# WarranWeng/ESR

Hardware: AMD Instinct MI355X
Metric: SR event-frames/sec (whole node), 2x NFS-syn (higher is better)
Workload: dtype bf16; 1 GPU; model=ESRNet-basech8, global_batch=64, seq_len=8, seqn=3, window_events=2048, input=128x128->256x256, scale=2, upsampler=pixelshuffle, hip_graphs=full, parallelism=dp1

## Files before the change

### esr_amd/ops/conv.py

```python

from __future__ import annotations

import os

import torch
import torch.nn.functional as F

from .native import get_ext

__all__ = ["conv2d_act", "native_conv_supported", "ACT_IDS"]

ACT_IDS = {None: 0, "none": 0, "relu": 1, "sigmoid": 2, "tanh": 3}

stats = {"native_calls": 0, "native_calls_fp16": 0, "native_bias_grad": 0}

_MFMA_MIN_COUT = 32
_CIK = 32


_FP16_DEFAULT = "1"


_BIAS_GRAD_DEFAULT = "native"


def _enabled() -> bool:
    return os.environ.get("ESR_NATIVE_CONV", "1") != "0"


def _native_bias_grad() -> bool:
    return os.environ.get("ESR_BIAS_GRAD", _BIAS_GRAD_DEFAULT) != "aten"


def native_fp16_enabled() -> bool:
    return os.environ.get("ESR_NATIVE_FP16", _FP16_DEFAULT) != "0"


def compute_dtype(autocast_on: bool, autocast_dtype, x_dtype,
                  fp16_enabled: bool | None = None):
    dt = autocast_dtype if autocast_on else x_dtype
    if dt == torch.bfloat16:
        return torch.bfloat16
    if dt == torch.float16:
        if fp16_enabled is None:
            fp16_enabled = native_fp16_enabled()
        return torch.float16 if fp16_enabled else None
    return None


def _ceil(v: int, m: int) -> int:
    return (v + m - 1) // m * m


def _pack(w: torch.Tensor) -> torch.Tensor:
    O, I, k, _ = w.shape
    t = w.permute(2, 3, 0, 1).reshape(k * k, O, I)
    op, ip = _ceil(O, 16), _ceil(I, _CIK)
    if op != O or ip != I:
        t = F.pad(t, (0, ip - I, 0, op - O))
    return t.contiguous()


class _NativeConv2dFn(torch.autograd.Function):
    @staticmethod
    def forward(ctx, x, w, bias, stride, act_id):
        ext = get_ext()
        ks = w.shape[2]
        cout, cin = w.shape[0], w.shape[1]
        bias_f = bias.float() if bias is not None else None
        if cout >= _MFMA_MIN_COUT:
            y = ext.conv2d_fwd_mfma(x, _pack(w), bias_f, cout, ks, stride,
                                    act_id)
        elif cin < _MFMA_MIN_COUT and x.shape[-1] % 8 == 0:
            y = ext.conv2d_fwd_valu2(x, w.contiguous(), bias_f, stride,
                                     act_id)
        else:
            y = ext.conv2d_fwd_valu(x, w.contiguous(), bias_f, stride, act_id)
        ctx.save_for_backward(x, w, y)
        ctx.stride_ = stride
        ctx.act_id = act_id
        ctx.has_bias = bias is not None
        return y

    @staticmethod
    def backward(ctx, dy):
        ext = get_ext()
        x, w, y = ctx.saved_tensors
        stride, act_id = ctx.stride_, ctx.act_id
        ks = w.shape[2]
        cout, cin = w.shape[0], w.shape[1]
        dy = dy.contiguous()
        fused_db = ctx.has_bias and _native_bias_grad()
        db = None
        if fused_db:
            stats["native_bias_grad"] += 1
            if act_id:
                dpre, db = ext.act_grad_bias(dy, y, act_id)[:2]
            else:
                dpre, db = dy, ext.bias_grad(dy)[0]
        else:
            dpre = ext.act_grad(dy, y, act_id) if act_id else dy
        aten_db = ctx.has_bias and not fused_db

        mode = os.environ.get("ESR_CONV_BWD", "aten")
        native_bwd = mode == "native" or (
            mode == "auto" and stride == 1 and cin >= _MFMA_MIN_COUT)
        if x.dtype != torch.bfloat16:
            native_bwd = False
        if not native_bwd:
            dx, dw, db_aten = torch.ops.aten.convolution_backward(
                dpre, x, w, [cout] if aten_db else None,
                [stride, stride], [ks // 2, ks // 2], [1, 1], False, [0, 0],
                1, [True, True, aten_db])
            return dx, dw, db_aten if aten_db else db, None, None

        if stride == 1:
            wt = w.transpose(0, 1)
            if ks == 3:
                wt = wt.flip((2, 3))
            if cin >= _MFMA_MIN_COUT:
                dx = ext.conv2d_fwd_mfma(dpre, _pack(wt), None, cin, ks, 1, 0)
            else:
                dx = ext.conv2d_fwd_valu(dpre, wt.contiguous(), None, 1, 0)
        else:
            dx = ext.conv2d_dgrad_s2(dpre, w.contiguous(),
                                     x.shape[2], x.shape[3])

        dwp = ext.conv2d_wgrad_mfma(x, dpre, ks, stride,
                                    _ceil(cin, 16), _ceil(cout, 16))
        dw = dwp.permute(1, 0, 2, 3)[:cout, :cin].to(w.dtype)
        if aten_db:
            db = dpre.sum(dim=(0, 2, 3), dtype=torch.float32).to(w.dtype)
        return dx, dw, db, None, None


def shape_supported(conv: torch.nn.Conv2d, dtype=None) -> bool:
    if conv.out_channels < _MFMA_MIN_COUT and conv.in_channels < _MFMA_MIN_COUT:
        if conv.stride[0] != 1:
            return False
    if dtype == torch.float16:
        if conv.out_channels < _MFMA_MIN_COUT <= conv.in_channels:
            return False
        if conv.out_channels >= 128 and conv.kernel_size == (3, 3) \
                and conv.stride == (1, 1):
            return False
    if conv.groups != 1 or conv.dilation != (1, 1):
        return False
    kh, kw = conv.kernel_size
    sh, sw = conv.stride
    ph, pw = conv.padding if isinstance(conv.padding, tuple) else \
        (conv.padding, conv.padding)
    if kh != kw or sh != sw or ph != pw:
        return False
    if (kh, sh) not in ((3, 1), (3, 2), (1, 1)):
        return False
    if ph != kh // 2:
        return False
    return True


def native_conv_supported(x: torch.Tensor, conv: torch.nn.Conv2d,
                          dtype=None) -> bool:
    if not (_enabled() and x.is_cuda and get_ext() is not None):
        return False
    return shape_supported(conv, dtype)


def conv2d_act(x: torch.Tensor, conv: torch.nn.Conv2d, act: str | None):
    if act not in ACT_IDS or not (x.is_cuda and _enabled()):
        return None
    autocast_on = torch.is_autocast_enabled()
    dt = compute_dtype(
        autocast_on,
        torch.get_autocast_dtype("cuda") if autocast_on else None, x.dtype)
    if dt is None or not native_conv_supported(x, conv, dt):
        return None
    if x.dtype != dt:
        x = x.to(dt)
    w, b = conv.weight, conv.bias
    if w.dtype != dt:
        w = w.to(dt)
        if b is not None:
            b = b.to(dt)
    stats["native_calls"] += 1
    if dt == torch.float16:
        stats["native_calls_fp16"] += 1
# ... 3 lines not shown
```

### esr_amd/ops/native/src/bindings.cpp

```cpp
#include <torch/extension.h>

at::Tensor deform_conv2d_forward(
    const at::Tensor&, const at::Tensor&, const at::Tensor&,
    const at::Tensor&, const c10::optional<at::Tensor>&,
    int64_t, int64_t, int64_t, int64_t, int64_t, int64_t, int64_t);
std::vector<at::Tensor> deform_conv2d_backward(
    const at::Tensor&, const at::Tensor&, const at::Tensor&,
    const at::Tensor&, const at::Tensor&,
    int64_t, int64_t, int64_t, int64_t, int64_t, int64_t, int64_t);
std::vector<at::Tensor> deform_conv2d_forward_cols(
    const at::Tensor&, const at::Tensor&, const at::Tensor&,
    const at::Tensor&, const c10::optional<at::Tensor>&,
    int64_t, int64_t, int64_t, int64_t, int64_t, int64_t, int64_t);
std::vector<at::Tensor> deform_conv2d_backward_cols(
    const at::Tensor&, const at::Tensor&, const at::Tensor&,
    const at::Tensor&, const at::Tensor&, const c10::optional<at::Tensor>&,
    int64_t, int64_t, int64_t, int64_t, int64_t, int64_t, int64_t,
    const std::string&);
at::Tensor deform_conv2d_forward_fused(
    const at::Tensor&, const at::Tensor&, const at::Tensor&,
    const at::Tensor&, const c10::optional<at::Tensor>&, int64_t);
at::Tensor deform_im2col_debug(
    const at::Tensor&, const at::Tensor&, const at::Tensor&,
    int64_t, int64_t, int64_t, int64_t, int64_t, int64_t, int64_t, int64_t,
    int64_t);

std::vector<at::Tensor> gru_gates_ur_forward(const at::Tensor&,
                                             const at::Tensor&);
std::vector<at::Tensor> gru_gates_ur_backward(
    const at::Tensor&, const at::Tensor&, const at::Tensor&,
    const at::Tensor&, const at::Tensor&, const at::Tensor&);
std::vector<at::Tensor> gru_gates_out_forward(const at::Tensor&,
                                              const at::Tensor&,
                                              const at::Tensor&);
std::vector<at::Tensor> gru_gates_out_backward(
    const at::Tensor&, const at::Tensor&, const at::Tensor&,
    const at::Tensor&);

at::Tensor splat_count(const at::Tensor&, int64_t, int64_t);
at::Tensor splat_stack(const at::Tensor&, int64_t, int64_t, int64_t, double,
                       double);
int64_t grid_cap();

at::Tensor conv2d_fwd_mfma(const at::Tensor&, const at::Tensor&,
                           const c10::optional<at::Tensor>&,
                           int64_t, int64_t, int64_t, int64_t);
at::Tensor conv2d_fwd_valu(const at::Tensor&, const at::Tensor&,
                           const c10::optional<at::Tensor>&, int64_t, int64_t);
at::Tensor conv2d_fwd_valu2(const at::Tensor&, const at::Tensor&,
                            const c10::optional<at::Tensor>&, int64_t, int64_t);
at::Tensor conv2d_dgrad_s2(const at::Tensor&, const at::Tensor&,
                           int64_t, int64_t);
at::Tensor conv2d_wgrad_mfma(const at::Tensor&, const at::Tensor&,
                             int64_t, int64_t, int64_t, int64_t);
at::Tensor act_grad(const at::Tensor&, const at::Tensor&, int64_t);
std::vector<at::Tensor> act_grad_bias(const at::Tensor&, const at::Tensor&,
                                      int64_t, bool);
std::vector<at::Tensor> bias_grad(const at::Tensor&, bool);
int64_t bias_grad_chain(int64_t, int64_t, int64_t);
int64_t bias_grad_chunk();
at::Tensor gemm16_probe(const at::Tensor&, const at::Tensor&);

std::vector<at::Tensor> redistribute_stack_hip(const at::Tensor&, int64_t,
                                               int64_t, int64_t, int64_t);

void flat_grad_finite_check(const at::Tensor&, at::Tensor&);
void flat_adam_step(at::Tensor&, const at::Tensor&, at::Tensor&, at::Tensor&,
                    const c10::optional<at::Tensor>&, const at::Tensor&,
                    double, double, double, double, bool);
void flat_scale_update(at::Tensor&, bool, double, double, int64_t, double,
                       double);
void flat_grad_stats(const at::Tensor&, at::Tensor&, at::Tensor&, at::Tensor&,
                     double);
void flat_adam_step_clipped(at::Tensor&, const at::Tensor&, at::Tensor&,
                            at::Tensor&, const c10::optional<at::Tensor>&,
                            const at::Tensor&, const at::Tensor&, double,
                            double, double, double, bool);

void stream_window_advance(at::Tensor&, const at::Tensor&);
void stream_splat_ragged(const at::Tensor&, const at::Tensor&,
                         const at::Tensor&, at::Tensor&, int64_t);

void evs_batch_splat(const at::Tensor&, const at::Tensor&, at::Tensor&,
                     int64_t, int64_t, int64_t);
int64_t evs_batch_splat_chunk();

at::Tensor restoration_metrics(const at::Tensor&, const at::Tensor&, double);
std::vector<int64_t> restoration_metrics_tile();

std::vector<at::Tensor> sr_emit_scratch(const at::Tensor&, int64_t, int64_t);
at::Tensor sr_emit_counts(const at::Tensor&, int64_t);
void sr_emit_window(const at::Tensor&, const at::Tensor&,
                    const std::vector<at::Tensor>&, at::Tensor&, int64_t,
                    int64_t, int64_t, int64_t,
                    const std::vector<at::Tensor>&);

PYBIND11_MODULE(TORCH_EXTENSION_NAME, m) {
  m.def("deform_conv2d_forward", &deform_conv2d_forward,
        "modulated deformable conv forward (gfx950)");
  m.def("deform_conv2d_backward", &deform_conv2d_backward,
        "modulated deformable conv backward (gfx950, batched)");
  m.def("deform_conv2d_forward_cols", &deform_conv2d_forward_cols,
        "im2col + GEMM forward; returns (out, cols) for the backward to reuse");
  m.def("deform_conv2d_backward_cols", &deform_conv2d_backward_cols,
        "backward with optional saved columns and a path selector "
        "(auto / fused / split)");
  m.def("deform_im2col", &deform_im2col_debug,
        "deformable im2col (test hook)");
  m.def("deform_conv2d_forward_fused", &deform_conv2d_forward_fused,
        "fused im2col+MFMA deformable conv forward (test hook)");
  m.def("gru_gates_ur_forward", &gru_gates_ur_forward);
  m.def("gru_gates_ur_backward", &gru_gates_ur_backward);
  m.def("gru_gates_out_forward", &gru_gates_out_forward);
  m.def("gru_gates_out_backward", &gru_gates_out_backward);
  m.def("splat_count", &splat_count);
  m.def("splat_stack", &splat_stack);
  m.def("grid_cap", &grid_cap,
        "work items one grid of a capped grid-stride kernel covers");
  m.def("conv2d_fwd_mfma", &conv2d_fwd_mfma,
        "bf16/fp16 NCHW conv fwd, MFMA implicit GEMM, fused bias+act (gfx950)");
  m.def("conv2d_fwd_valu", &conv2d_fwd_valu,
        "bf16/fp16 NCHW conv fwd, direct VALU, fused bias+act (gfx950)");
  m.def("conv2d_fwd_valu2", &conv2d_fwd_valu2,
        "bf16/fp16 NCHW conv fwd, register-strip VALU v2 for tiny channels");
  m.def("conv2d_dgrad_s2", &conv2d_dgrad_s2,
        "bf16 stride-2 conv input-grad (gfx950)");
  m.def("conv2d_wgrad_mfma", &conv2d_wgrad_mfma,
        "bf16 conv weight-grad, MFMA split-K + fp32 atomics (gfx950)");
  m.def("act_grad", &act_grad, "fused activation backward (bf16/fp16)");
  m.def("act_grad_bias", &act_grad_bias,
        "activation backward + per-channel bias grad in one pass: "
        "{dpre, db}, with want_f32 also the fp32 sums; deterministic "
        "(bf16/fp16)",
        py::arg("dy"), py::arg("y"), py::arg("act"),
        py::arg("want_f32") = false);
  m.def("bias_grad", &bias_grad,
        "per-channel sum of an NCHW gradient: {db}, with want_f32 also the "
        "fp32 sums; deterministic (bf16/fp16)",
        py::arg("dy"), py::arg("want_f32") = false);
  m.def("bias_grad_chunk", &bias_grad_chunk,
        "elements of a channel one block of bias_grad sums");
  m.def("bias_grad_chain", &bias_grad_chain,
        "longest fp32 addition chain of bias_grad for (B, H, W)");
  m.def("gemm16_probe", &gemm16_probe, "16x16x32 bf16/fp16 MFMA fragment probe");
  m.def("redistribute_stack_hip", &redistribute_stack_hip,
        "count stack -> sorted event cloud, device-only "
        "(scan + scatter + segmented radix sort)");
  m.def("flat_grad_finite_check", &flat_grad_finite_check,
        "raise found_inf in the device state if the flat fp32 grad has "
        "inf/NaN");
  m.def("flat_adam_step", &flat_adam_step,
        "flat-buffer Adam/AdamW step with device-side un-scale and skip");
  m.def("flat_scale_update", &flat_scale_update,
        "GradScaler-style scale/step update of the device state");
  m.def("flat_grad_stats", &flat_grad_stats,
        "finite check plus deterministic fp64 sum of squares of the flat "
        "grad; writes grad norm, clip coefficient and clipped-step count");
  m.def("flat_adam_step_clipped", &flat_adam_step_clipped,
        "flat_adam_step with the gradient multiplied by the clip "
        "coefficient after un-scaling");
  m.def("stream_window_advance", &stream_window_advance,
        "per-stream sliding-window shift/reset of a [seqn,S,2,kH,kW] buffer, "
        "control read from a device tensor");
  m.def("stream_splat_ragged", &stream_splat_ragged,
        "splat concatenated per-stream LR event windows into the newest "
        "frame of a [seqn,S,2,kH,kW] buffer");
  m.def("evs_batch_splat", &evs_batch_splat,
        "splat a batch of packed event windows (jobs read from a device "
        "tensor) into [J,2,kH,kW] count planes, in place");
  m.def("evs_batch_splat_chunk", &evs_batch_splat_chunk,
        "events one block of evs_batch_splat covers");
  m.def("restoration_metrics", &restoration_metrics,
        "per-plane sum|p-t|, sum(p-t)^2, max t, min t and 7x7 SSIM sum of "
        "fp32 [P,H,W] maps, fp64 [P,5], deterministic");
  m.def("restoration_metrics_tile", &restoration_metrics_tile,
        "(TH, TW) pixel tile one block of restoration_metrics owns");
  m.def("sr_emit_scratch", &sr_emit_scratch,
        "scratch of sr_emit_window for (ncells, capacity), allocated once");
  m.def("sr_emit_counts", &sr_emit_counts,
        "the counts stage of sr_emit_window: NaN -> 0, else "
        "clamp(rint(v), 0, cell_cap), int32 (test hook)");
// ... 7 lines not shown
```

### esr_amd/ops/native/src/conv2d.hip

```cpp

#include <torch/extension.h>
#include <ATen/hip/HIPContext.h>
#include "esr_common.h"

namespace {

using s16x8 = __attribute__((ext_vector_type(8))) short;
using f32x4 = __attribute__((ext_vector_type(4))) float;

constexpr int TW = 32;
constexpr int TH = 2;
constexpr int CIK = 32;
constexpr int SLOT = 40;

template <int ACT> ESR_INLINE float apply_act(float v);
template <> ESR_INLINE float apply_act<0>(float v) { return v; }
template <> ESR_INLINE float apply_act<1>(float v) { return v > 0.f ? v : 0.f; }
template <> ESR_INLINE float apply_act<2>(float v) { return esr_sigmoid(v); }
template <> ESR_INLINE float apply_act<3>(float v) { return tanhf(v); }

ESR_INLINE float bf16u_to_f(ushort u) {
  unsigned int x = (unsigned int)u << 16;
  return __uint_as_float(x);
}
// ... 76 lines not shown
        for (int c = 0; c < CIK; ++c)
          vals[c] = (c < cmax) ? src[c * plane] : (ushort)0;
      } else {
#pragma unroll
        for (int c = 0; c < CIK; ++c) vals[c] = 0;
      }
#pragma unroll
      for (int v = 0; v < CIK / 8; ++v)
        *reinterpret_cast<s16x8*>(&patch[p * SLOT + v * 8]) =
            *reinterpret_cast<const s16x8*>(&vals[v * 8]);
    }
    __syncthreads();

#pragma unroll
    for (int tap = 0; tap < KS * KS; ++tap) {
      const int ky = tap / KS, kx = tap % KS;
      s16x8 a[MREP];
#pragma unroll
      for (int m = 0; m < MREP; ++m) {
        int row = co0 + wm * 16 * MREP + m * 16 + (lane & 15);
        row = row < Cout_p ? row : Cout_p - 1;
        a[m] = *reinterpret_cast<const s16x8*>(
            &wp[((long long)tap * Cout_p + row) * Cin_p + ci0 + kgrp]);
      }
#pragma unroll
      for (int nf = 0; nf < 2; ++nf) {
        const int pidx = wn * 32 + nf * 16 + (lane & 15);
        const int py = (pidx >> 5) * STRIDE + ky;
        const int px = (pidx & 31) * STRIDE + kx;
        const s16x8 bfrag = *reinterpret_cast<const s16x8*>(
            &patch[(py * PW + px) * SLOT + kgrp]);
#pragma unroll
        for (int m = 0; m < MREP; ++m)
          acc[m][nf] = E::mfma(a[m], bfrag, acc[m][nf]);
      }
    }
  }

#pragma unroll
  for (int m = 0; m < MREP; ++m) {
#pragma unroll
    for (int nf = 0; nf < 2; ++nf) {
      const int pidx = wn * 32 + nf * 16 + (lane & 15);
      const int oy = ty0 + (pidx >> 5), ox = tx0 + (pidx & 31);
      if (oy >= Ho || ox >= Wo) continue;
#pragma unroll
      for (int j = 0; j < 4; ++j) {
        const int co = co0 + wm * 16 * MREP + m * 16 + (lane >> 4) * 4 + j;
        if (co >= Cout) continue;
        float v = acc[m][nf][j];
        if (bias) v += bias[co];
        v = apply_act<ACT>(v);
        y[(((long long)b * Cout + co) * Ho + oy) * Wo + ox] = E::from_f(v);
      }
    }
  }
}


template <typename E, int KS, int STRIDE, int ACT>
__global__ void conv2d_fwd_valu_kernel(
    long long n, const ushort* __restrict__ x,
    const ushort* __restrict__ w,
    const float* __restrict__ bias, ushort* __restrict__ y,
    int Cin, int H, int W, int Cout, int Ho, int Wo) {
  constexpr int PAD = KS / 2;
  ESR_KERNEL_LOOP(i, n) {
    const int ox = (int)(i % Wo);
    long long t = i / Wo;
    const int oy = (int)(t % Ho); t /= Ho;
    const int co = (int)(t % Cout);
    const int b = (int)(t / Cout);
    const long long plane = (long long)H * W;
    const ushort* xb = x + (long long)b * Cin * plane;
    const ushort* wc = w + (long long)co * Cin * KS * KS;
    float acc = bias ? bias[co] : 0.f;
    const int iy0 = oy * STRIDE - PAD, ix0 = ox * STRIDE - PAD;
    for (int ci = 0; ci < Cin; ++ci) {
      const ushort* xp = xb + ci * plane;
      const ushort* wk = wc + ci * KS * KS;
#pragma unroll
      for (int ky = 0; ky < KS; ++ky) {
        const int iy = iy0 + ky;
        if (iy < 0 || iy >= H) continue;
#pragma unroll
        for (int kx = 0; kx < KS; ++kx) {
          const int ix = ix0 + kx;
          if (ix < 0 || ix >= W) continue;
          acc += E::to_f(xp[(long long)iy * W + ix]) *
                 E::to_f(wk[ky * KS + kx]);
        }
      }
    }
    y[i] = E::from_f(apply_act<ACT>(acc));
  }
}


template <typename E, int KS, int STRIDE, int ACT, int COCH>
__global__ __launch_bounds__(256)
void conv2d_fwd_valu2_kernel(
    const ushort* __restrict__ x,
    const ushort* __restrict__ w,
    const float* __restrict__ bias, ushort* __restrict__ y,
    int Cin, int H, int W, int Cout, int Ho, int Wo,
    long long nstrips, int nsx) {
// ... 362 lines not shown
            const int slot = KS == 1 ? oy % NSLOT
                : (((oy + ky - PAD) % NSLOT) + NSLOT) % NSLOT;
#pragma unroll
            for (int nci = 0; nci < 2; ++nci) {
              const s16x8 bfrag = *reinterpret_cast<const s16x8*>(
                  &xs[((nci * 16 + (lane & 15)) * NSLOT + slot) * WGV2_XW
                      + kgrp]);
#pragma unroll
              for (int kx = 0; kx < KS; ++kx)
                acc[ky * KS + kx][nci] =
                    __builtin_amdgcn_mfma_f32_16x16x32_bf16(
                        afrag[kx], bfrag, acc[ky * KS + kx][nci], 0, 0, 0);
            }
          }
        }
      }
      __syncthreads();
    }
  }

  if (abl == 1) return;
  float* part = dwp + ((((long long)blockIdx.x * gridDim.y + blockIdx.y)
                        * gridDim.z + blockIdx.z) * (32 * 64 * NTAP));
#pragma unroll
  for (int tap = 0; tap < NTAP; ++tap) {
#pragma unroll
    for (int nci = 0; nci < 2; ++nci) {
#pragma unroll
      for (int j = 0; j < 4; ++j) {
        const int co = wave * 16 + (lane >> 4) * 4 + j;
        const int ci = nci * 16 + (lane & 15);
        part[((long long)ci * 64 + co) * NTAP + tap] = acc[tap][nci][j];
      }
    }
  }
}

template <int NTAP>
__global__ void conv2d_wgrad_reduce_kernel(
    long long n, const float* __restrict__ part, int ng, int ciblks,
    int coblks, int Cin_p, int Cout_p, float* __restrict__ dwp) {
  ESR_KERNEL_LOOP(i, n) {
    const int tap = (int)(i % NTAP);
    const int co = (int)((i / NTAP) % Cout_p);
    const int ci = (int)(i / ((long long)NTAP * Cout_p));
    const int cib = ci / 32, cob = co / 64;
    const long long base =
        ((long long)cib * coblks + cob) * (32 * 64 * NTAP)
        + (((long long)(ci % 32) * 64 + (co % 64)) * NTAP + tap);
    const long long gstride = (long long)ciblks * coblks * (32 * 64 * NTAP);
    float v = 0.f;
    for (int g = 0; g < ng; ++g) v += part[g * gstride + base];
    dwp[i] = v;
  }
}


template <int ACT> ESR_INLINE float act_grad_value(float g, float v) {
  if (ACT == 0) return g;
  if (ACT == 1) return v > 0.f ? g : 0.f;
  if (ACT == 2) return g * v * (1.f - v);
  return g * (1.f - v * v);
}

template <typename E, int ACT>
ESR_INLINE ushort act_grad_elem(ushort dy, ushort y) {
  float d = act_grad_value<ACT>(E::to_f(dy), E::to_f(y));
  asm("" : "+v"(d));
  return E::from_f(d);
}

template <typename E, int ACT>
__global__ void act_grad_kernel(long long n, const ushort* __restrict__ dy,
                                const ushort* __restrict__ y,
                                ushort* __restrict__ dpre) {
  ESR_KERNEL_LOOP(i, n) {
    dpre[i] = act_grad_elem<E, ACT>(dy[i], y[i]);
  }
}


constexpr int BG_VPT = 2;
constexpr int BG_CHUNK = ESR_BLOCK * BG_VPT * 8;

ESR_INLINE float bg_block_sum(float v, float* red) {
#pragma unroll
  for (int off = 32; off > 0; off >>= 1) v += __shfl_down(v, off, 64);
  const int lane = threadIdx.x & 63, wave = threadIdx.x >> 6;
  __syncthreads();
  if (lane == 0) red[wave] = v;
  __syncthreads();
  return ((red[0] + red[1]) + red[2]) + red[3];
}

template <typename E, int ACT, bool STORE>
__global__ __launch_bounds__(ESR_BLOCK)
void act_grad_bias_kernel(int C, unsigned int HW, unsigned int L,
                          unsigned int P, bool vec,
                          const ushort* __restrict__ dy,
                          const ushort* __restrict__ y,
                          ushort* __restrict__ dpre,
                          float* __restrict__ part) {
  __shared__ float red[ESR_BLOCK / 64];
  const long long nitem = (long long)C * P;
  for (long long item = blockIdx.x; item < nitem; item += gridDim.x) {
    const int c = (int)(item / P);
// ... 128 lines not shown
  if (!bias.has_value()) return nullptr;
  TORCH_CHECK(bias->scalar_type() == at::kFloat && bias->is_contiguous() &&
              bias->device() == x.device(),
              "bias: contiguous fp32 tensor on x's device required, got ",
              bias->scalar_type());
  return bias->data_ptr<float>();
}

at::Tensor conv2d_fwd_mfma(const at::Tensor& x, const at::Tensor& wp,
                           const c10::optional<at::Tensor>& bias,
                           int64_t Cout, int64_t ks, int64_t stride,
                           int64_t act) {
  check_16bit(x, "conv2d_fwd_mfma: x");
  check_16bit(wp, "conv2d_fwd_mfma: wp");
  check_same_dtype(x, wp, "conv2d_fwd_mfma: x / wp");
  TORCH_CHECK(x.dim() == 4 && wp.dim() == 3,
              "x [B,Cin,H,W], wp: packed [ntap,Cop,Cip]");
  const int B = x.size(0), Cin = x.size(1), H = x.size(2), W = x.size(3);
  const int Cout_p = wp.size(1), Cin_p = wp.size(2);
  TORCH_CHECK(wp.size(0) == ks * ks && Cin_p % CIK == 0 && Cout_p % 16 == 0);
  const int Ho = (H + 2 * (int)(ks / 2) - (int)ks) / (int)stride + 1;
  const int Wo = (W + 2 * (int)(ks / 2) - (int)ks) / (int)stride + 1;
  auto y = at::empty({B, Cout, Ho, Wo}, x.options());
  const float* bias_ptr = bias_ptr_f32(bias, x);
  const int mrep = (Cout > 32 && Cout_p % 32 == 0) ? 2 : 1;
  const int ntx = (Wo + TW - 1) / TW, nty = (Ho + TH - 1) / TH;
  dim3 grid(ntx * nty, B, (Cout_p + 32 * mrep - 1) / (32 * mrep));
  auto stream = at::hip::getCurrentHIPStream();
  DISPATCH_ELEM(x.scalar_type(), [&] {
  DISPATCH_KS_STRIDE((int)ks, (int)stride, [&] {
    DISPATCH_ACT((int)act, [&] {
      if (mrep == 2)
        hipLaunchKernelGGL((conv2d_fwd_mfma_kernel<elem_t, kKS, kST, kAct, 2>),
                           grid, dim3(256), 0, stream,
                           (const ushort*)x.data_ptr(), (const ushort*)wp.data_ptr(),
                           bias_ptr, (ushort*)y.data_ptr(),
                           Cin, H, W, (int)Cout, Ho, Wo, Cin_p, Cout_p, ntx);
      else
        hipLaunchKernelGGL((conv2d_fwd_mfma_kernel<elem_t, kKS, kST, kAct, 1>),
                           grid, dim3(256), 0, stream,
                           (const ushort*)x.data_ptr(), (const ushort*)wp.data_ptr(),
                           bias_ptr, (ushort*)y.data_ptr(),
                           Cin, H, W, (int)Cout, Ho, Wo, Cin_p, Cout_p, ntx);
      return 0;
    });
    return 0;
  });
  return 0;
  });
  C10_HIP_KERNEL_LAUNCH_CHECK();
  return y;
}

at::Tensor conv2d_fwd_valu(const at::Tensor& x, const at::Tensor& w,
                           const c10::optional<at::Tensor>& bias,
                           int64_t stride, int64_t act) {
  check_16bit(x, "conv2d_fwd_valu: x");
  check_16bit(w, "conv2d_fwd_valu: w");
  check_same_dtype(x, w, "conv2d_fwd_valu: x / w");
  const int B = x.size(0), Cin = x.size(1), H = x.size(2), W = x.size(3);
  const int Cout = w.size(0), ks = w.size(2);
  const int Ho = (H + 2 * (ks / 2) - ks) / (int)stride + 1;
  const int Wo = (W + 2 * (ks / 2) - ks) / (int)stride + 1;
  auto y = at::empty({B, Cout, Ho, Wo}, x.options());
  const float* bias_ptr = bias_ptr_f32(bias, x);
  const long long n = (long long)B * Cout * Ho * Wo;
  auto stream = at::hip::getCurrentHIPStream();
  DISPATCH_ELEM(x.scalar_type(), [&] {
  DISPATCH_KS_STRIDE(ks, (int)stride, [&] {
    DISPATCH_ACT((int)act, [&] {
      hipLaunchKernelGGL((conv2d_fwd_valu_kernel<elem_t, kKS, kST, kAct>),
                         dim3(esr_grid(n)), dim3(ESR_BLOCK), 0, stream,
                         n, (const ushort*)x.data_ptr(), (const ushort*)w.data_ptr(),
                         bias_ptr, (ushort*)y.data_ptr(), Cin, H, W, Cout, Ho, Wo);
      return 0;
    });
    return 0;
  });
  return 0;
  });
  C10_HIP_KERNEL_LAUNCH_CHECK();
  return y;
}

at::Tensor conv2d_fwd_valu2(const at::Tensor& x, const at::Tensor& w,
                            const c10::optional<at::Tensor>& bias,
                            int64_t stride, int64_t act) {
  check_16bit(x, "conv2d_fwd_valu2: x");
  check_16bit(w, "conv2d_fwd_valu2: w");
  check_same_dtype(x, w, "conv2d_fwd_valu2: x / w");
  const int B = x.size(0), Cin = x.size(1), H = x.size(2), W = x.size(3);
  const int Cout = w.size(0), ks = w.size(2);
  TORCH_CHECK(Cin <= 32, "valu2 is for tiny-channel shapes (Cin <= 32)");
  const int Ho = (H + 2 * (ks / 2) - ks) / (int)stride + 1;
  const int Wo = (W + 2 * (ks / 2) - ks) / (int)stride + 1;
  auto y = at::empty({B, Cout, Ho, Wo}, x.options());
  const float* bias_ptr = bias_ptr_f32(bias, x);
  const int coch = Cout >= 8 || Cout > 2 ? 8 : 2;
  const int nsx = (Wo + 7) / 8;
  const long long nstrips = (long long)B * Ho * nsx;
  dim3 grid(esr_grid(nstrips), 1, (Cout + coch - 1) / coch);
  auto stream = at::hip::getCurrentHIPStream();
  DISPATCH_ELEM(x.scalar_type(), [&] {
  DISPATCH_KS_STRIDE(ks, (int)stride, [&] {
    DISPATCH_ACT((int)act, [&] {
      if (coch == 8)
        hipLaunchKernelGGL((conv2d_fwd_valu2_kernel<elem_t, kKS, kST, kAct, 8>),
                           grid, dim3(256), 0, stream,
                           (const ushort*)x.data_ptr(),
                           (const ushort*)w.data_ptr(), bias_ptr,
                           (ushort*)y.data_ptr(), Cin, H, W, Cout, Ho, Wo,
                           nstrips, nsx);
      else
        hipLaunchKernelGGL((conv2d_fwd_valu2_kernel<elem_t, kKS, kST, kAct, 2>),
                           grid, dim3(256), 0, stream,
                           (const ushort*)x.data_ptr(),
                           (const ushort*)w.data_ptr(), bias_ptr,
                           (ushort*)y.data_ptr(), Cin, H, W, Cout, Ho, Wo,
                           nstrips, nsx);
      return 0;
    });
    return 0;
  });
  return 0;
  });
  C10_HIP_KERNEL_LAUNCH_CHECK();
  return y;
}

at::Tensor conv2d_dgrad_s2(const at::Tensor& dy, const at::Tensor& w,
                           int64_t H, int64_t W) {
  check_bf16_4d(dy, "conv2d_dgrad_s2: dy");
  check_bf16_4d(w, "conv2d_dgrad_s2: w");
  const int B = dy.size(0), Cout = dy.size(1), Ho = dy.size(2), Wo = dy.size(3);
  const int Cin = w.size(1), ks = w.size(2);
  TORCH_CHECK(ks == 3, "dgrad_s2 supports 3x3 only");
  auto dx = at::empty({B, Cin, H, W}, dy.options());
  const long long n = (long long)B * Cin * H * W;
  auto stream = at::hip::getCurrentHIPStream();
  hipLaunchKernelGGL((conv2d_dgrad_s2_valu_kernel<3>),
                     dim3(esr_grid(n)), dim3(ESR_BLOCK), 0, stream,
                     n, (const ushort*)dy.data_ptr(), (const ushort*)w.data_ptr(),
                     (ushort*)dx.data_ptr(), Cin, (int)H, (int)W, Cout, Ho, Wo);
  C10_HIP_KERNEL_LAUNCH_CHECK();
  return dx;
}

at::Tensor conv2d_wgrad_mfma(const at::Tensor& x, const at::Tensor& dpre,
                             int64_t ks, int64_t stride,
                             int64_t Cin_p, int64_t Cout_p) {
  check_bf16_4d(x, "conv2d_wgrad: x");
  check_bf16_4d(dpre, "conv2d_wgrad: dpre");
  const int B = x.size(0), Cin = x.size(1), H = x.size(2), W = x.size(3);
  const int Cout = dpre.size(1), Ho = dpre.size(2), Wo = dpre.size(3);
  TORCH_CHECK(Cin_p % 16 == 0 && Cout_p % 16 == 0);
  auto dwp = at::zeros({Cin_p, Cout_p, ks, ks},
                       x.options().dtype(at::kFloat));
  const int uw = (W + TW - 1) / TW;
  auto stream = at::hip::getCurrentHIPStream();
  if (stride == 1) {
    const int ciblks = (Cin_p + 31) / 32, coblks = (Cout_p + 63) / 64;
    long long nb = (long long)B * uw * ciblks * coblks;
    int fpb = 1;
    while (fpb < 32 && fpb * 2 <= B && nb / (fpb * 2) >= 1024) fpb *= 2;
    static const int abl = [] {
      const char* e = getenv("ESR_WGRAD_ABL");
      return e ? atoi(e) : 0;
    }();
    const int bblks = (B + fpb - 1) / fpb;
    const int ng = bblks * uw;
    const int ntap = (int)(ks * ks);
    dim3 grid((unsigned)ng, ciblks, coblks);
    auto part = at::empty({(long long)ng * ciblks * coblks * 32 * 64 * ntap},
                          x.options().dtype(at::kFloat));
    if (ks == 3)
      hipLaunchKernelGGL((conv2d_wgrad_s1_kernel<3>), grid, dim3(256), 0,
                         stream, (const ushort*)x.data_ptr(),
                         (const ushort*)dpre.data_ptr(),
                         part.data_ptr<float>(),
                         Cin, H, W, Cout, (int)Cin_p, (int)Cout_p, uw, B,
                         fpb, abl);
    else
      hipLaunchKernelGGL((conv2d_wgrad_s1_kernel<1>), grid, dim3(256), 0,
                         stream, (const ushort*)x.data_ptr(),
                         (const ushort*)dpre.data_ptr(),
                         part.data_ptr<float>(),
                         Cin, H, W, Cout, (int)Cin_p, (int)Cout_p, uw, B,
                         fpb, abl);
    const long long nred = (long long)Cin_p * Cout_p * ntap;
    if (ks == 3)
      hipLaunchKernelGGL((conv2d_wgrad_reduce_kernel<9>),
                         dim3(esr_grid(nred)), dim3(ESR_BLOCK), 0, stream,
                         nred, part.data_ptr<float>(), ng, ciblks, coblks,
                         (int)Cin_p, (int)Cout_p, dwp.data_ptr<float>());
    else
      hipLaunchKernelGGL((conv2d_wgrad_reduce_kernel<1>),
                         dim3(esr_grid(nred)), dim3(ESR_BLOCK), 0, stream,
                         nred, part.data_ptr<float>(), ng, ciblks, coblks,
                         (int)Cin_p, (int)Cout_p, dwp.data_ptr<float>());
  } else {
    const int rows_per_blk = 16;
    const long long nslab =
        (long long)B * ((Ho + rows_per_blk - 1) / rows_per_blk) * uw;
    dim3 grid((unsigned)nslab, Cin_p / 16, Cout_p / 16);
    TORCH_CHECK(ks == 3, "stride-2 wgrad supports 3x3 only");
    hipLaunchKernelGGL((conv2d_wgrad_mfma_kernel<3, 2>),
                       grid, dim3(256), 0, stream,
                       (const ushort*)x.data_ptr(), (const ushort*)dpre.data_ptr(),
                       dwp.data_ptr<float>(), Cin, H, W, Cout, Ho, Wo,
                       (int)Cin_p, (int)Cout_p, rows_per_blk);
  }
  C10_HIP_KERNEL_LAUNCH_CHECK();
  return dwp;
}

at::Tensor act_grad(const at::Tensor& dy, const at::Tensor& y, int64_t act) {
  check_16bit(dy, "act_grad: dy");
  check_16bit(y, "act_grad: y");
  check_same_dtype(dy, y, "act_grad: dy / y");
  TORCH_CHECK(dy.numel() == y.numel(), "act_grad: dy and y sizes differ");
  auto dpre = at::empty_like(dy);
  const long long n = dy.numel();
  auto stream = at::hip::getCurrentHIPStream();
  DISPATCH_ELEM(dy.scalar_type(), [&] {
  DISPATCH_ACT((int)act, [&] {
    if (kAct == 0) { dpre.copy_(dy); return 0; }
    hipLaunchKernelGGL((act_grad_kernel<elem_t, kAct>),
                       dim3(esr_grid(n)), dim3(ESR_BLOCK), 0, stream,
                       n, (const ushort*)dy.data_ptr(),
                       (const ushort*)y.data_ptr(), (ushort*)dpre.data_ptr());
    return 0;
  });
  return 0;
  });
  C10_HIP_KERNEL_LAUNCH_CHECK();
  return dpre;
}

int64_t bias_grad_chunk() { return BG_CHUNK; }

int64_t bias_grad_chain(int64_t B, int64_t H, int64_t W) {
// ... 98 lines not shown
```

Measured before the change: 3099 frames/s.

## Add stride-1 MFMA conv core and route deep convs' forward and backward natively

Result: faster. 3605 frames/s (median of 6 runs) (+16.3%).

```diff
diff --git a/esr_amd/ops/conv.py b/esr_amd/ops/conv.py
--- a/esr_amd/ops/conv.py
+++ b/esr_amd/ops/conv.py
@@ -22,6 +22,12 @@
 
 
 _BIAS_GRAD_DEFAULT = "native"
+
+
+_CONV_BWD_DEFAULT = "auto"
+_AUTO_WGRAD_MIN_CIN = 192
+
+_CONV_FWD_DEFAULT = "auto"
 
 
 def _enabled() -> bool:
@@ -68,7 +74,10 @@
         ks = w.shape[2]
         cout, cin = w.shape[0], w.shape[1]
         bias_f = bias.float() if bias is not None else None
-        if cout >= _MFMA_MIN_COUT:
+        if fwd_core_route(os.environ.get("ESR_CONV_FWD", _CONV_FWD_DEFAULT),
+                          x.dtype == torch.bfloat16, ks, stride, cin, cout):
+            y = ext.conv2d_s1(x, w.contiguous(), bias_f, act_id, False)
+        elif cout >= _MFMA_MIN_COUT:
             y = ext.conv2d_fwd_mfma(x, _pack(w), bias_f, cout, ks, stride,
                                     act_id)
         elif cin < _MFMA_MIN_COUT and x.shape[-1] % 8 == 0:
@@ -102,36 +111,63 @@
             dpre = ext.act_grad(dy, y, act_id) if act_id else dy
         aten_db = ctx.has_bias and not fused_db
 
-        mode = os.environ.get("ESR_CONV_BWD", "aten")
-        native_bwd = mode == "native" or (
-            mode == "auto" and stride == 1 and cin >= _MFMA_MIN_COUT)
-        if x.dtype != torch.bfloat16:
-            native_bwd = False
-        if not native_bwd:
+        dgrad_native, wgrad_native = bwd_route(
+            os.environ.get("ESR_CONV_BWD", _CONV_BWD_DEFAULT),
+            x.dtype == torch.bfloat16, ks, stride, cin, cout)
+        pad = [ks // 2, ks // 2]
+        if not (dgrad_native and wgrad_native):
             dx, dw, db_aten = torch.ops.aten.convolution_backward(
                 dpre, x, w, [cout] if aten_db else None,
-                [stride, stride], [ks // 2, ks // 2], [1, 1], False, [0, 0],
-                1, [True, True, aten_db])
-            return dx, dw, db_aten if aten_db else db, None, None
-
-        if stride == 1:
-            wt = w.transpose(0, 1)
-            if ks == 3:
-                wt = wt.flip((2, 3))
-            if cin >= _MFMA_MIN_COUT:
-                dx = ext.conv2d_fwd_mfma(dpre, _pack(wt), None, cin, ks, 1, 0)
+                [stride, stride], pad, [1, 1], False, [0, 0], 1,
+                [not dgrad_native, not wgrad_native, aten_db])
+            if aten_db:
+                db = db_aten
+        elif aten_db:
+            db = dpre.sum(dim=(0, 2, 3), dtype=torch.float32).to(w.dtype)
+
+        if dgrad_native:
+            if stride == 1 and cin >= _MFMA_MIN_COUT:
+                dx = ext.conv2d_s1(dpre, w.contiguous(), None, 0, True)
+            elif stride == 1:
+                wt = w.transpose(0, 1)
+                if ks == 3:
+                    wt = wt.flip((2, 3))
+                dx = ext.conv2d_fwd_valu(dpre, wt.contiguous(), None, 1, 0)
             else:
-                dx = ext.conv2d_fwd_valu(dpre, wt.contiguous(), None, 1, 0)
-        else:
-            dx = ext.conv2d_dgrad_s2(dpre, w.contiguous(),
-                                     x.shape[2], x.shape[3])
-
-        dwp = ext.conv2d_wgrad_mfma(x, dpre, ks, stride,
-                                    _ceil(cin, 16), _ceil(cout, 16))
-        dw = dwp.permute(1, 0, 2, 3)[:cout, :cin].to(w.dtype)
-        if aten_db:
-            db = dpre.sum(dim=(0, 2, 3), dtype=torch.float32).to(w.dtype)
+                dx = ext.conv2d_dgrad_s2(dpre, w.contiguous(),
+                                         x.shape[2], x.shape[3])
+        if wgrad_native:
+            if stride == 1:
+                dw = ext.conv2d_wgrad_s1(x, dpre, ks)
+            else:
+                dwp = ext.conv2d_wgrad_mfma(x, dpre, ks, stride,
+                                            _ceil(cin, 16), _ceil(cout, 16))
+                dw = dwp.permute(1, 0, 2, 3)[:cout, :cin].to(w.dtype)
         return dx, dw, db, None, None
+
+
+def bwd_route(mode: str, is_bf16: bool, ks: int, stride: int, cin: int,
+              cout: int) -> tuple[bool, bool]:
+    if not is_bf16 or mode == "aten":
+        return False, False
+    if mode == "native":
+        return True, True
+    if mode == "dgrad":
+        return True, False
+    deep_s1 = stride == 1 and ks in (1, 3) and \
+        cin >= _MFMA_MIN_COUT and cout >= _MFMA_MIN_COUT
+    if not deep_s1 or ks != 3:
+        return False, False
+    return True, cin >= _AUTO_WGRAD_MIN_CIN
+
+
+def fwd_core_route(mode: str, is_bf16: bool, ks: int, stride: int, cin: int,
+                   cout: int) -> bool:
+    if mode == "mfma" or not is_bf16:
+        return False
+    deep_s1 = stride == 1 and ks in (1, 3) and \
+        cin >= _MFMA_MIN_COUT and cout >= _MFMA_MIN_COUT
+    return deep_s1
 
 
 def shape_supported(conv: torch.nn.Conv2d, dtype=None) -> bool:
diff --git a/esr_amd/ops/native/src/bindings.cpp b/esr_amd/ops/native/src/bindings.cpp
--- a/esr_amd/ops/native/src/bindings.cpp
+++ b/esr_amd/ops/native/src/bindings.cpp
@@ -53,6 +53,9 @@
                            int64_t, int64_t);
 at::Tensor conv2d_wgrad_mfma(const at::Tensor&, const at::Tensor&,
                              int64_t, int64_t, int64_t, int64_t);
+at::Tensor conv2d_s1(const at::Tensor&, const at::Tensor&,
+                     const c10::optional<at::Tensor>&, int64_t, bool);
+at::Tensor conv2d_wgrad_s1(const at::Tensor&, const at::Tensor&, int64_t);
 at::Tensor act_grad(const at::Tensor&, const at::Tensor&, int64_t);
 std::vector<at::Tensor> act_grad_bias(const at::Tensor&, const at::Tensor&,
                                       int64_t, bool);
@@ -127,6 +130,12 @@
         "bf16 stride-2 conv input-grad (gfx950)");
   m.def("conv2d_wgrad_mfma", &conv2d_wgrad_mfma,
         "bf16 conv weight-grad, MFMA split-K + fp32 atomics (gfx950)");
+  m.def("conv2d_s1", &conv2d_s1,
+        "bf16/fp16 stride-1 3x3/1x1 conv, 8x32-tile MFMA core: forward with "
+        "fused bias+act, or the input grad (dgrad=True) (gfx950)");
+  m.def("conv2d_wgrad_s1", &conv2d_wgrad_s1,
+        "bf16 stride-1 conv weight grad, deterministic two-stage reduction, "
+        "dW [Cout,Cin,k,k] bf16 (gfx950)");
   m.def("act_grad", &act_grad, "fused activation backward (bf16/fp16)");
   m.def("act_grad_bias", &act_grad_bias,
         "activation backward + per-channel bias grad in one pass: "
diff --git a/esr_amd/ops/native/src/conv2d.hip b/esr_amd/ops/native/src/conv2d.hip
--- a/esr_amd/ops/native/src/conv2d.hip
+++ b/esr_amd/ops/native/src/conv2d.hip
@@ -152,6 +152,221 @@
         if (bias) v += bias[co];
         v = apply_act<ACT>(v);
         y[(((long long)b * Cout + co) * Ho + oy) * Wo + ox] = E::from_f(v);
+      }
+    }
+  }
+}
+
+
+constexpr int C_TH = 8;
+
+ESR_INLINE float apply_act_rt(float v, int act) {
+  switch (act) {
+    case 1: return apply_act<1>(v);
+    case 2: return apply_act<2>(v);
+    case 3: return apply_act<3>(v);
+    default: return v;
+  }
+}
+
+__global__ void conv2d_pack_w_kernel(
+    long long n, const ushort* __restrict__ w,
+    ushort* __restrict__ wp,
+    int O, int I, int KS, int Mp, int Kp, int dgrad) {
+  ESR_KERNEL_LOOP(i, n) {
+    const int k = (int)(i % Kp);
+    const int m = (int)((i / Kp) % Mp);
+    const int tap = (int)(i / ((long long)Kp * Mp));
+    const int ky = tap / KS, kx = tap % KS;
+    const int o = dgrad ? k : m, ci = dgrad ? m : k;
+    const int sy = dgrad ? KS - 1 - ky : ky, sx = dgrad ? KS - 1 - kx : kx;
+    wp[i] = (o < O && ci < I)
+        ? w[(((long long)o * I + ci) * KS + sy) * KS + sx] : (ushort)0;
+  }
+}
+
+template <typename E, int KS, int MC>
+__global__ __launch_bounds__(256, 2)
+void conv2d_s1_core_kernel(
+    const ushort* __restrict__ x,
+    const ushort* __restrict__ wp,
+    const float* __restrict__ bias,
+    ushort* __restrict__ y,
+    int Cin, int H, int W, int Cout, int Kp, int Mp, int ntx, int act,
+    int valign) {
+  constexpr int PAD = KS / 2;
+  constexpr int PH = C_TH + 2 * PAD;
+  constexpr int PWC = TW + 2 * PAD;
+  constexpr int MCW = MC / 2;
+  constexpr int BUF = PH * PWC * SLOT;
+  constexpr int NV = PH * 4 * 4;
+  constexpr int NHALO = PAD ? PH * 4 * 2 : 0;
+  static_assert(NV + NHALO <= 256, "one staging unit per thread");
+  __shared__ __attribute__((aligned(16))) ushort patch[2 * BUF];
+
+  const int tid = threadIdx.x;
+  const int lane = tid & 63;
+  const int wave = tid >> 6;
+  const int wm = wave >> 1, wn = wave & 1;
+  const int l15 = lane & 15, lg = lane >> 4;
+
+  const int ty0 = (blockIdx.x / ntx) * C_TH;
+  const int tx0 = (blockIdx.x % ntx) * TW;
+  const int b = blockIdx.y;
+  const int co0 = blockIdx.z * (16 * MC);
+
+  const long long plane = (long long)H * W;
+  const ushort* xb = x + (long long)b * Cin * plane;
+
+  const bool is_vec = tid < NV;
+  const bool is_halo = !is_vec && tid < NV + NHALO;
+  int u_row, u_cg, u_px;
+  int u_col;
+  if (is_vec) {
+    const int g = tid & 3;
+    u_row = (tid >> 2) % PH;
+    u_cg = tid / (4 * PH);
+    u_px = tx0 + g * 8;
+    u_col = PAD + g * 8;
+  } else {
+    const int h = tid - NV;
+    const int side = h & 1;
+    u_row = (h >> 1) % PH;
+    u_cg = (h >> 1) / PH;
+    u_px = side ? tx0 + TW : tx0 - 1;
+    u_col = side ? PWC - 1 : 0;
+  }
+  const int u_iy = ty0 - PAD + u_row;
+  const bool u_row_ok = u_iy >= 0 && u_iy < H;
+  const bool u_vec_ok = valign && u_px + 8 <= W;
+  const ushort* u_src = xb + (long long)u_iy * W + u_px;
+
+  s16x8 pre[8];
+
+  auto load_chunk = [&](int ci0) {
+    if (is_vec) {
+#pragma unroll
+      for (int j = 0; j < 8; ++j) {
+        const int c = ci0 + u_cg * 8 + j;
+        s16x8 v = {};
+        if (c < Cin && u_row_ok) {
+          const ushort* src = u_src + c * plane;
+          if (u_vec_ok) {
+            v = *reinterpret_cast<const s16x8*>(src);
+          } else {
+#pragma unroll
+            for (int e = 0; e < 8; ++e)
+              v[e] = (u_px + e < W) ? (short)src[e] : (short)0;
+          }
+        }
+        pre[j] = v;
+      }
+    } else if (is_halo) {
+      s16x8 v = {};
+      if (u_row_ok && u_px >= 0 && u_px < W) {
+#pragma unroll
+        for (int j = 0; j < 8; ++j) {
+          const int c = ci0 + u_cg * 8 + j;
+          v[j] = (c < Cin) ? (short)u_src[c * plane] : (short)0;
+        }
+      }
+      pre[0] = v;
+    }
+  };
+
+  auto store_chunk = [&](ushort* buf) {
+    ushort* dst = buf + (u_row * PWC + u_col) * SLOT + u_cg * 8;
+    if (is_vec) {
+#pragma unroll
+      for (int e = 0; e < 8; ++e) {
+        s16x8 v;
+#pragma unroll
+        for (int j = 0; j < 8; ++j) v[j] = pre[j][e];
+        *reinterpret_cast<s16x8*>(dst + e * SLOT) = v;
+      }
+    } else if (is_halo) {
+      *reinterpret_cast<s16x8*>(dst) = pre[0];
+    }
+  };
+
+  f32x4 acc[8][MCW] = {};
+  const int kgrp = lg * 8;
+  const int nchunks = Kp / CIK;
+
+  load_chunk(0);
+  store_chunk(patch);
+  for (int ck = 0; ck < nchunks; ++ck) {
+    __syncthreads();
+    const ushort* cur = patch + (ck & 1) * BUF;
+    const bool more = ck + 1 < nchunks;
+    if (more) load_chunk((ck + 1) * CIK);
+
+    const int ci0 = ck * CIK;
+#pragma unroll 1
+    for (int ky = 0; ky < KS; ++ky)
+#pragma unroll
+    for (int kx = 0; kx < KS; ++kx) {
+      const int tap = ky * KS + kx;
+      s16x8 wf[MCW];
+#pragma unroll
+      for (int m = 0; m < MCW; ++m) {
+        const int row = co0 + (wm * MCW + m) * 16 + l15;
+        wf[m] = *reinterpret_cast<const s16x8*>(
+            &wp[((long long)tap * Mp + row) * Kp + ci0 + kgrp]);
+      }
+#pragma unroll
+      for (int nf = 0; nf < 8; ++nf) {
+        const int r = wn * 4 + (nf >> 1);
+        const int col = (nf & 1) * 16 + l15;
+        const s16x8 pf = *reinterpret_cast<const s16x8*>(
+            &cur[((r + ky) * PWC + col + kx) * SLOT + kgrp]);
+#pragma unroll
+        for (int m = 0; m < MCW; ++m)
+          acc[nf][m] = E::mfma(pf, wf[m], acc[nf][m]);
+      }
+    }
+    if (more) store_chunk(patch + ((ck + 1) & 1) * BUF);
+  }
+
+  const bool odd = lg & 1;
+  const int ox0 = tx0 + (odd ? 16 : 0) + (lg >> 1) * 8;
+#pragma unroll
+  for (int m = 0; m < MCW; ++m) {
+    const int co = co0 + (wm * MCW + m) * 16 + l15;
+    const float bv = (bias && co < Cout) ? bias[co] : 0.f;
+#pragma unroll
+    for (int r = 0; r < 4; ++r) {
+      unsigned int p[2][2];
+#pragma unroll
+      for (int h = 0; h < 2; ++h)
+#pragma unroll
+        for (int q = 0; q < 2; ++q) {
+          const ushort lo =
+              E::from_f(apply_act_rt(acc[2 * r + h][m][2 * q] + bv, act));
+          const ushort hi =
+              E::from_f(apply_act_rt(acc[2 * r + h][m][2 * q + 1] + bv, act));
+          p[h][q] = (unsigned int)lo | ((unsigned int)hi << 16);
+        }
+      const unsigned int s0 = odd ? p[0][0] : p[1][0];
+      const unsigned int s1 = odd ? p[0][1] : p[1][1];
+      const unsigned int r0 = (unsigned int)__shfl_xor((int)s0, 16, 64);
+      const unsigned int r1 = (unsigned int)__shfl_xor((int)s1, 16, 64);
+      unsigned int o[4];
+      o[0] = odd ? r0 : p[0][0];
+      o[1] = odd ? r1 : p[0][1];
+      o[2] = odd ? p[1][0] : r0;
+      o[3] = odd ? p[1][1] : r1;
+      const int oy = ty0 + wn * 4 + r;
+      if (co < Cout && oy < H && ox0 < W) {
+        ushort* dst = y + (((long long)b * Cout + co) * H + oy) * W + ox0;
+        if (valign && ox0 + 8 <= W) {
+          *reinterpret_cast<uint4*>(dst) = make_uint4(o[0], o[1], o[2], o[3]);
+        } else {
+#pragma unroll
+          for (int e = 0; e < 8; ++e)
+            if (ox0 + e < W)
+              dst[e] = (ushort)(o[e >> 1] >> ((e & 1) * 16));
+        }
       }
     }
   }
@@ -620,6 +835,24 @@
     float v = 0.f;
     for (int g = 0; g < ng; ++g) v += part[g * gstride + base];
     dwp[i] = v;
+  }
+}
+
+template <int NTAP>
+__global__ void conv2d_wgrad_reduce_out_kernel(
+    long long n, const float* __restrict__ part, int ng, int coblks,
+    int Cin, int Cout, ushort* __restrict__ dw) {
+  ESR_KERNEL_LOOP(i, n) {
+    const int tap = (int)(i % NTAP);
+    const int co64 = (int)((i / NTAP) % 64);
+    const int ci32 = (int)((i / (NTAP * 64)) % 32);
+    const int blk = (int)(i / (NTAP * 64 * 32));
+    const int ci = (blk / coblks) * 32 + ci32;
+    const int co = (blk % coblks) * 64 + co64;
+    if (ci >= Cin || co >= Cout) continue;
+    float v = 0.f;
+    for (int g = 0; g < ng; ++g) v += part[g * n + i];
+    dw[((long long)co * Cin + ci) * NTAP + tap] = f_to_bf16u(v);
   }
 }
 
@@ -854,6 +1087,69 @@
   return y;
 }
 
+at::Tensor conv2d_s1(const at::Tensor& x, const at::Tensor& w,
+                     const c10::optional<at::Tensor>& bias, int64_t act,
+                     bool dgrad) {
+  check_16bit(x, "conv2d_s1: x");
+  check_16bit(w, "conv2d_s1: w");
+  check_same_dtype(x, w, "conv2d_s1: x / w");
+  TORCH_CHECK(x.dim() == 4 && w.dim() == 4 && w.size(2) == w.size(3),
+              "conv2d_s1: x [B,C,H,W], w [O,I,k,k]");
+  const int ks = w.size(2);
+  TORCH_CHECK(ks == 1 || ks == 3, "conv2d_s1: 3x3 or 1x1 only, got ", ks);
+  TORCH_CHECK(act >= 0 && act <= 3, "conv2d_s1: act id ", act);
+  TORCH_CHECK(!dgrad || (!bias.has_value() && act == 0),
+              "conv2d_s1: the input grad takes no bias or activation");
+  const int O = w.size(0), I = w.size(1);
+  const int B = x.size(0), K = x.size(1), H = x.size(2), W = x.size(3);
+  const int M = dgrad ? I : O;
+  TORCH_CHECK(K == (dgrad ? O : I), "conv2d_s1: x has ", K,
+              " channels, w wants ", dgrad ? O : I);
+  TORCH_CHECK(B <= 65535, "conv2d_s1: batch above the grid's y limit");
+  const int mfr = (M + 15) / 16;
+  const int nsplit = (mfr + 7) / 8;
+  const int mc = ((mfr + nsplit - 1) / nsplit + 1) / 2 * 2;
+  const int Mp = nsplit * mc * 16;
+  const int Kp = (K + CIK - 1) / CIK * CIK;
+  const float* bias_ptr = bias_ptr_f32(bias, x);
+  if (bias_ptr) TORCH_CHECK(bias->numel() == M, "conv2d_s1: bias size");
+  auto wp = at::empty({ks * ks, Mp, Kp}, w.options());
+  auto y = at::empty({B, M, H, W}, x.options());
+  const int valign = W % 8 == 0 && (uintptr_t)x.data_ptr() % 16 == 0 &&
+                     (uintptr_t)y.data_ptr() % 16 == 0;
+  const int ntx = (W + TW - 1) / TW, nty = (H + C_TH - 1) / C_TH;
+  dim3 grid(ntx * nty, B, nsplit);
+  auto stream = at::hip::getCurrentHIPStream();
+  const long long npack = (long long)ks * ks * Mp * Kp;
+  hipLaunchKernelGGL(conv2d_pack_w_kernel, dim3(esr_grid(npack)),
+                     dim3(ESR_BLOCK), 0, stream, npack,
+                     (const ushort*)w.data_ptr(), (ushort*)wp.data_ptr(),
+                     O, I, ks, Mp, Kp, (int)dgrad);
+  DISPATCH_ELEM(x.scalar_type(), [&] {
+    auto launch = [&](auto kern) {
+      hipLaunchKernelGGL(kern, grid, dim3(256), 0, stream,
+                         (const ushort*)x.data_ptr(),
+                         (const ushort*)wp.data_ptr(), bias_ptr,
+                         (ushort*)y.data_ptr(), K, H, W, M, Kp, Mp, ntx,
+                         (int)act, valign);
+    };
+    auto by_mc = [&](auto ks_tag) {
+      constexpr int kKS = decltype(ks_tag)::value;
+      switch (mc) {
+        case 2: launch(conv2d_s1_core_kernel<elem_t, kKS, 2>); break;
+        case 4: launch(conv2d_s1_core_kernel<elem_t, kKS, 4>); break;
+        case 6: launch(conv2d_s1_core_kernel<elem_t, kKS, 6>); break;
+        default: launch(conv2d_s1_core_kernel<elem_t, kKS, 8>); break;
+      }
+    };
+    if (ks == 3) by_mc(std::integral_constant<int, 3>{});
+    else by_mc(std::integral_constant<int, 1>{});
+    return 0;
+  });
+  C10_HIP_KERNEL_LAUNCH_CHECK();
+  return y;
+}
+
 at::Tensor conv2d_fwd_valu(const at::Tensor& x, const at::Tensor& w,
                            const c10::optional<at::Tensor>& bias,
                            int64_t stride, int64_t act) {
@@ -948,6 +1244,71 @@
   return dx;
 }
 
+static at::Tensor wgrad_s1_stage1(const at::Tensor& x, const at::Tensor& dpre,
+                                  int ks, int Cin_p, int Cout_p, int* ng_out) {
+  const int B = x.size(0), Cin = x.size(1), H = x.size(2), W = x.size(3);
+  const int Cout = dpre.size(1);
+  const int uw = (W + TW - 1) / TW;
+  const int ciblks = (Cin_p + 31) / 32, coblks = (Cout_p + 63) / 64;
+  long long nb = (long long)B * uw * ciblks * coblks;
+  int fpb = 1;
+  while (fpb < 32 && fpb * 2 <= B && nb / (fpb * 2) >= 1024) fpb *= 2;
+  static const int abl = [] {
+    const char* e = getenv("ESR_WGRAD_ABL");
+    return e ? atoi(e) : 0;
+  }();
+  const int bblks = (B + fpb - 1) / fpb;
+  const int ng = bblks * uw;
+  const int ntap = ks * ks;
+  dim3 grid((unsigned)ng, ciblks, coblks);
+  auto part = at::empty({(long long)ng * ciblks * coblks * 32 * 64 * ntap},
+                        x.options().dtype(at::kFloat));
+  auto stream = at::hip::getCurrentHIPStream();
+  if (ks == 3)
+    hipLaunchKernelGGL((conv2d_wgrad_s1_kernel<3>), grid, dim3(256), 0,
+                       stream, (const ushort*)x.data_ptr(),
+                       (const ushort*)dpre.data_ptr(),
+                       part.data_ptr<float>(),
+                       Cin, H, W, Cout, Cin_p, Cout_p, uw, B, fpb, abl);
+  else
+    hipLaunchKernelGGL((conv2d_wgrad_s1_kernel<1>), grid, dim3(256), 0,
+                       stream, (const ushort*)x.data_ptr(),
+                       (const ushort*)dpre.data_ptr(),
+                       part.data_ptr<float>(),
+                       Cin, H, W, Cout, Cin_p, Cout_p, uw, B, fpb, abl);
+  *ng_out = ng;
+  return part;
+}
+
+at::Tensor conv2d_wgrad_s1(const at::Tensor& x, const at::Tensor& dpre,
+                           int64_t ks) {
+  check_bf16_4d(x, "conv2d_wgrad_s1: x");
+  check_bf16_4d(dpre, "conv2d_wgrad_s1: dpre");
+  TORCH_CHECK(ks == 1 || ks == 3, "conv2d_wgrad_s1: 3x3 or 1x1 only");
+  TORCH_CHECK(x.size(0) == dpre.size(0) && x.size(2) == dpre.size(2) &&
+              x.size(3) == dpre.size(3), "conv2d_wgrad_s1: x / dpre shapes");
+  const int Cin = x.size(1), Cout = dpre.size(1);
+  const int Cin_p = (Cin + 15) / 16 * 16, Cout_p = (Cout + 15) / 16 * 16;
+  const int ciblks = (Cin_p + 31) / 32, coblks = (Cout_p + 63) / 64;
+  int ng = 0;
+  auto part = wgrad_s1_stage1(x, dpre, (int)ks, Cin_p, Cout_p, &ng);
+  auto dw = at::empty({Cout, Cin, ks, ks}, x.options());
+  const long long n = (long long)ciblks * coblks * 32 * 64 * ks * ks;
+  auto stream = at::hip::getCurrentHIPStream();
+  if (ks == 3)
+    hipLaunchKernelGGL((conv2d_wgrad_reduce_out_kernel<9>),
+                       dim3(esr_grid(n)), dim3(ESR_BLOCK), 0, stream, n,
+                       part.data_ptr<float>(), ng, coblks, Cin, Cout,
+                       (ushort*)dw.data_ptr());
+  else
+    hipLaunchKernelGGL((conv2d_wgrad_reduce_out_kernel<1>),
+                       dim3(esr_grid(n)), dim3(ESR_BLOCK), 0, stream, n,
+                       part.data_ptr<float>(), ng, coblks, Cin, Cout,
+                       (ushort*)dw.data_ptr());
+  C10_HIP_KERNEL_LAUNCH_CHECK();
+  return dw;
+}
+
 at::Tensor conv2d_wgrad_mfma(const at::Tensor& x, const at::Tensor& dpre,
                              int64_t ks, int64_t stride,
                              int64_t Cin_p, int64_t Cout_p) {
@@ -962,33 +1323,10 @@
   auto stream = at::hip::getCurrentHIPStream();
   if (stride == 1) {
     const int ciblks = (Cin_p + 31) / 32, coblks = (Cout_p + 63) / 64;
-    long long nb = (long long)B * uw * ciblks * coblks;
-    int fpb = 1;
-    while (fpb < 32 && fpb * 2 <= B && nb / (fpb * 2) >= 1024) fpb *= 2;
-    static const int abl = [] {
-      const char* e = getenv("ESR_WGRAD_ABL");
-      return e ? atoi(e) : 0;
-    }();
-    const int bblks = (B + fpb - 1) / fpb;
-    const int ng = bblks * uw;
     const int ntap = (int)(ks * ks);
-    dim3 grid((unsigned)ng, ciblks, coblks);
-    auto part = at::empty({(long long)ng * ciblks * coblks * 32 * 64 * ntap},
-                          x.options().dtype(at::kFloat));
-    if (ks == 3)
-      hipLaunchKernelGGL((conv2d_wgrad_s1_kernel<3>), grid, dim3(256), 0,
-                         stream, (const ushort*)x.data_ptr(),
-                         (const ushort*)dpre.data_ptr(),
-                         part.data_ptr<float>(),
-                         Cin, H, W, Cout, (int)Cin_p, (int)Cout_p, uw, B,
-                         fpb, abl);
-    else
-      hipLaunchKernelGGL((conv2d_wgrad_s1_kernel<1>), grid, dim3(256), 0,
-                         stream, (const ushort*)x.data_ptr(),
-                         (const ushort*)dpre.data_ptr(),
-                         part.data_ptr<float>(),
-                         Cin, H, W, Cout, (int)Cin_p, (int)Cout_p, uw, B,
-                         fpb, abl);
+    int ng = 0;
+    auto part = wgrad_s1_stage1(x, dpre, (int)ks, (int)Cin_p, (int)Cout_p,
+                                &ng);
     const long long nred = (long long)Cin_p * Cout_p * ntap;
     if (ks == 3)
       hipLaunchKernelGGL((conv2d_wgrad_reduce_kernel<9>),
```
